# PimLb/POMDP_PBVI_Exploration

Measured on AMD Instinct MI355X. Metric: alpha-vector backups/sec, higher is better.
Workload: dtype f32

## Files before the change

include/pbvi_hip.h:

```cpp
#ifndef PBVI_HIP_H
#define PBVI_HIP_H

#include <stddef.h>
#include <stdint.h>

#ifdef __cplusplus
extern "C" {
#endif

typedef struct pbvi_engine pbvi_engine_t;

enum pbvi_status {
    PBVI_OK = 0,
    PBVI_EINVAL = -1,
    PBVI_ENOMEM = -2,
    PBVI_ERUNTIME = -3,
    PBVI_EUNSUPPORTED = -4
};

enum pbvi_dtype { PBVI_F32 = 0, PBVI_F64 = 1 };

enum pbvi_mode {
    PBVI_SPARSE = 0,
    PBVI_DENSE = 1
// ... 158 lines not shown
int pbvi_set_score_split(pbvi_engine_t* e, int mode);

int pbvi_set_gamma_tiling(pbvi_engine_t* e, int mode, int64_t chunk_rows);
int pbvi_gamma_tiling_plan(int32_t S, int32_t A, int32_t O, int64_t V, int64_t B, int dtype, int64_t budget_bytes,
                           int64_t* chunk_rows, int64_t* n_chunks, int64_t* bytes_needed);

int pbvi_set_tie_window(pbvi_engine_t* e, double rel);

int pbvi_debug_poison(int enable);
int64_t pbvi_debug_alloc_limit(int64_t mb);
int pbvi_engine_after_oom(pbvi_engine_t* e);
int64_t pbvi_debug_live_bytes(void);

int pbvi_debug_gemm_dense(int enable);
int pbvi_debug_split_schedule(int schedule);
int64_t pbvi_debug_slabs(pbvi_engine_t* e, void* out, int64_t cap_bytes);
int pbvi_debug_slabs_fill(pbvi_engine_t* e, int byte);

int64_t pbvi_device_bytes(const pbvi_engine_t* e);

#ifdef __cplusplus
}
#endif
#endif
```

pomdp_pbvi_exploration_amd/csrc/engine.hip:

```cpp
#include <algorithm>
#include <atomic>
#include <cmath>
#include <cstddef>
#include <cstdio>
#include <cstdlib>
#include <cstring>
#include <condition_variable>
#include <mutex>
#include <new>
#include <string>
#include <thread>
#include <unistd.h>
#include <vector>

#include "backup_kernels.h"
#include "split_bf16.h"

namespace pbvi {

static thread_local std::string g_err;
static int g_poison = -1;
static bool poison_enabled() {
    if (g_poison < 0) g_poison = getenv("PBVI_POISON") != nullptr ? 1 : 0;
    return g_poison == 1;
}
void set_error(const std::string& msg) { g_err = msg; }

#define HIPCHK(expr)                                                                         \
    do {                                                                                     \
        hipError_t _e = (expr);                                                              \
        if (_e != hipSuccess) {                                                              \
// ... 753 lines not shown
    virtual int store_select(int which, const int32_t* ids, int64_t n) = 0;
    virtual int store_reset(int which) = 0;
    virtual int after_oom() = 0;
    virtual int belief_update(const int32_t* act, const int32_t* obs, void* out) = 0;
    virtual int beliefs_advance(const int32_t* act, const int32_t* obs, const uint8_t* keep, int64_t* out_B) = 0;
    virtual int beliefs_fetch(void* out) = 0;
    virtual int set_rto_f64(const double* rto) = 0;
    virtual int64_t belief_walk(const double* b0, int64_t n, const int32_t* act, const int32_t* obs, const uint8_t* restart,
                                double* out) = 0;
    virtual int64_t beliefs_count() const = 0;
    virtual int walk_keys(int64_t n, uint64_t* out_keys) = 0;
    virtual int backup_value_max(double* out_value) = 0;
    virtual int q_values(double gamma, double* out_q, int32_t* out_action, int32_t* out_best) = 0;
    virtual int64_t debug_slabs(void* out, int64_t cap_bytes) = 0;
    virtual int debug_slabs_fill(int byte) = 0;
    virtual int rollout(int source, const int32_t* alpha_actions, double gamma, const int32_t* start_states,
                        const uint8_t* end_mask, uint64_t first_sim_id, uint64_t seed, int64_t T, int32_t* out_states,
                        int32_t* out_actions, int32_t* out_observations, int32_t* out_steps) = 0;
    virtual int infotaxis(double* out_g, int32_t* out_action, double* out_p_obs, double* out_entropy) = 0;
    virtual int env_set_frames(const uint8_t* frames, int64_t F, int64_t C, const int32_t* channel_of_action) = 0;
    virtual int env_set_table(const double* obs_prob) = 0;
    virtual int env_clear() = 0;
    virtual int rollout_env(int source, const int32_t* alpha_actions, double gamma, const int32_t* start_states,
                            const uint8_t* end_mask, int end_observation, const int64_t* shifts, uint64_t first_sim_id,
                            uint64_t seed, int64_t T, int32_t* out_states, int32_t* out_actions, int32_t* out_observations,
                            int32_t* out_steps, uint8_t* out_lost) = 0;
};

template <typename T>
class EngineT : public EngineBase {
// ... 105 lines not shown
    DevBuf e_bv_{mem_}, e_bs_{mem_}, e_err_{mem_}, e_rdot_{mem_}, e_act_{mem_}, e_ares_{mem_}, e_bres_{mem_}, e_rep_{mem_}, e_uniq_{mem_}, e_inv_{mem_}, e_slotd_{mem_}, e_cnt_{mem_, DevBuf::MODEL}, e_out_{mem_}, e_slot_{mem_};
    hipEvent_t ev_early_[2] = {nullptr, nullptr};
    hipEvent_t ev_ids_ = nullptr;
    hipEvent_t ev_nzA_ = nullptr;
    DevBuf nzBw_{mem_, DevBuf::MODEL};
    DevBuf nzB_{mem_, DevBuf::MODEL}, nzA_{mem_}, klist_{mem_}, kcount_{mem_}, nchunks_{mem_}, need_{mem_}, skws_{mem_};
    DevBuf dense_{mem_, DevBuf::MODEL}, nzD_{mem_, DevBuf::MODEL}, nzAlpha_{mem_}, prod_{mem_}, klistD_{mem_}, kcountD_{mem_}, nchunksD_{mem_};
    int64_t rows_pad_s_ = 0, dense_pairs_ = 0;
    std::vector<int> h_kcountD_;
    PinnedBuf kc_pin_{pinned_, "hipHostFree(kcount)"};
    hipStream_t stream2_ = nullptr;
    hipStream_t stream3_ = nullptr;
    hipEvent_t ev_fork_ = nullptr, ev_join_ = nullptr, ev_lists_ = nullptr, ev_xr_[2] = {nullptr, nullptr};
    GemmPlan plan_ = {};
    int64_t slab_bytes_ = 0;
    hipEvent_t ev_[9] = {};
    hipEvent_t ev_pg_[2] = {};
    bool have_result_ = false, res_sorted_ = false;
    int64_t res_B_ = 0;
    int screen_mode_ = 1;
    int split_mode_ = 1;
    bool split_supported_ = false;
    int fuse_project_ = 1;
    double irr_frac_ = 0.0;
    DevBuf irr_{mem_, DevBuf::MODEL};
    DevBuf mat_{mem_}, vlist_{mem_};
    DevBuf ctile_{mem_};
    std::vector<int32_t> h_ctile_;
    int n_mat_ = 0;
    bool gam_pad_compact_ = false;
// ... 772 lines not shown
            HIPCHK(hipStreamSynchronize(stream_));
        }
        return PBVI_OK;
    }

    int64_t debug_slabs(void* out, int64_t cap_bytes) override {
        if (slab_bytes_ <= 0 || slabs_.p == nullptr || (int64_t)slabs_.cap < slab_bytes_)
            FAIL(PBVI_EINVAL, "debug_slabs: no score GEMM has run");
        if (!out) return slab_bytes_;
        if (cap_bytes < slab_bytes_) FAIL(PBVI_EINVAL, "debug_slabs: the output array is smaller than the slab buffer");
        HIPCHK(hipSetDevice(device_));
        HIPCHK(hipMemcpyAsync(out, slabs_.p, (size_t)slab_bytes_, hipMemcpyDeviceToHost, stream_));
        HIPCHK(hipStreamSynchronize(stream_));
        return slab_bytes_;
    }
    int debug_slabs_fill(int byte) override {
        if (slab_bytes_ <= 0 || slabs_.p == nullptr || (int64_t)slabs_.cap < slab_bytes_)
            FAIL(PBVI_EINVAL, "debug_slabs_fill: no score GEMM has run");
        HIPCHK(hipSetDevice(device_));
        HIPCHK(hipMemsetAsync(slabs_.p, byte & 0xff, (size_t)slab_bytes_, stream_));
        HIPCHK(hipStreamSynchronize(stream_));
        return PBVI_OK;
    }

    int beliefs_fetch(void* out) override {
        if (B_ <= 0) FAIL(PBVI_EINVAL, "beliefs_fetch: no belief block resident");
        if (!out) FAIL(PBVI_EINVAL, "beliefs_fetch: NULL argument");
        HIPCHK(hipSetDevice(device_));
        if (!sorted_) {
            HIPCHK(hipMemcpy2DAsync(out, (size_t)S_ * sizeof(T), bel_.p, (size_t)S_pad_ * sizeof(T), (size_t)S_ * sizeof(T),
// ... 994 lines not shown
    }
    if constexpr (kF32) {
        const int64_t n_pad = round_up(rows_y, GEMM_BN);
        if (m_pad > 0x7fffffff || n_pad > 0x7fffffff) FAIL(PBVI_EUNSUPPORTED, "score_gemm: operand rows exceed int32");
        plan_ = make_gemm_plan((int)m_pad, (int)n_pad, S_pad_);
        const size_t pairs = (size_t)plan_.tiles_m * plan_.tiles_n;
        if ((rc = slabs_.ensure((size_t)plan_.c_floats * sizeof(float)))) return rc;
        slab_bytes_ = (int64_t)plan_.c_floats * (int64_t)sizeof(float);
        if ((rc = klist_.ensure(pairs * plan_.k_tiles * sizeof(int)))) return rc;
        if ((rc = kcount_.ensure(pairs * sizeof(int)))) return rc;
        if ((rc = nchunks_.ensure(pairs * sizeof(int)))) return rc;
        if ((rc = skws_.ensure(streamk_workspace_ints(plan_) * sizeof(int)))) return rc;
        int sp = split != nullptr && *split && plan_.streamk && (fused == nullptr || fused->R == 1) ? 1 : 0;
        if (sp && (!own_block || !split_plane())) sp = 0;
        if (split != nullptr) *split = sp;
        HIPCHK(launch_gemm_nt_f32(sp ? belsp_.as<float>() : (const float*)X, S_pad_, (const float*)Y, S_pad_, slabs_.as<float>(), plan_,
                                  nzX, nzB, G, v_group, (int)rows_y, klist_.as<int>(), kcount_.as<int>(),
                                  nchunks_.as<int>(), stream_, 1, 0, 0, skws_.as<int>(), list_stream, ev_lists_, nullptr, nullptr,
                                  fused, sp));
        sv->slabs = slabs_.as<T>();
        sv->slab_stride = plan_.slab_stride;
        sv->ldc = plan_.ldc;
        sv->nchunks = nchunks_.as<int>();
        sv->tiles_m = plan_.tiles_m;
        sv->fixed = 0;
        sv->first_block = plan_.streamk ? skws_.as<int>() + (pairs + 1) + plan_.nblocks : nullptr;
    } else {
        const int kt32s = S_pad_ / GEMM_BK;
        const int split = f64_uses_mfma(m_rows, rows_y) ? gemm_f64_split((int)m_rows, (int)rows_y, kt32s) : 1;
        if ((rc = slabs_.ensure((size_t)split * m_rows * rows_y * sizeof(T)))) return rc;
// ... 5 lines not shown
        } else {
            const int kt32 = S_pad_ / GEMM_BK;
            if ((rc = klist_.ensure(gemm_f64_klist_ints((int)m_rows, (int)rows_y, kt32) * sizeof(int)))) return rc;
            if ((rc = kcount_.ensure(gemm_f64_kcount_ints((int)m_rows, (int)rows_y, kt32) * sizeof(int)))) return rc;
            HIPCHK(launch_gemm_nt_f64((const double*)X, S_pad_, (int)m_rows, (const double*)Y, S_pad_, (int)rows_y,
                                      slabs_.as<double>(), (int)rows_y, S_pad_, nzX, nzB, G, v_group, klist_.as<int>(),
                                      kcount_.as<int>(), stream_, split, m_rows * rows_y));
            f64_pairs_ = (int64_t)gemm_f64_pairs((int)m_rows, (int)rows_y);
        }
        sv->slabs = slabs_.as<T>();
        sv->slab_stride = 0;
        sv->ldc = (int)rows_y;
        sv->nchunks = nullptr;
        sv->tiles_m = 0;
        sv->fixed = 1;
    }
    return PBVI_OK;
}

template <typename T>
int EngineT<T>::project_dense(double gamma) {
    int rc;
    const int AO = A_ * O_;
    const int64_t Vt = V_, Vt_pad = round_up(Vt, GEMM_BM);
    int64_t ld_prod, batch_stride;
    if constexpr (kF32) {
        const int64_t n_pad = rows_pad_s_;
        GemmPlan pl = make_gemm_plan((int)Vt_pad, (int)n_pad, S_pad_, true);
        const size_t pairs = (size_t)pl.tiles_m * pl.tiles_n;
        ld_prod = n_pad;
// ... 1283 lines not shown
void* pbvi_host_alloc(size_t bytes) {
    void* p = nullptr;
    if (bytes == 0) return nullptr;
    if (hipHostMalloc(&p, bytes, hipHostMallocDefault) != hipSuccess) {
        (void)hipGetLastError();
        pbvi::set_error("pbvi_host_alloc: hipHostMalloc of " + std::to_string(bytes) + " bytes failed");
        return nullptr;
    }
    return p;
}
void pbvi_host_free(void* p) {
    if (p && hipHostFree(p) != hipSuccess) (void)hipGetLastError();
}
int pbvi_debug_gemm_dense(int enable) { return pbvi::set_gemm_force_dense(enable); }
int pbvi_debug_split_schedule(int schedule) { return pbvi::set_gemm_split_schedule(schedule); }
int64_t pbvi_debug_slabs(pbvi_engine_t* e, void* out, int64_t cap_bytes) {
    NEED(e);
    return e->impl->debug_slabs(out, cap_bytes);
}
int pbvi_debug_slabs_fill(pbvi_engine_t* e, int byte) {
    NEED(e);
    return e->impl->debug_slabs_fill(byte);
}
int pbvi_backup(pbvi_engine_t* e, const void* beliefs, int64_t B, double gamma, int flags, void* out_alpha,
                int32_t* out_action, int32_t* out_best_alpha, uint8_t* out_keep, pbvi_stats_t* stats) {
    NEED(e);
    int rc = e->impl->beliefs_set(beliefs, B);
    if (rc) return rc;
    rc = e->impl->backup_run(gamma, flags, stats);
    if (rc) return rc;
// ... 183 lines not shown
```

pomdp_pbvi_exploration_amd/csrc/gemm.hip:

```cpp
#include "pbvi_common.h"
#include "split_bf16.h"

#include <cstdlib>
#include <map>
#include <mutex>

namespace pbvi {

typedef float f32x4 __attribute__((ext_vector_type(4)));
typedef float f32x16 __attribute__((ext_vector_type(16)));

constexpr int TILE_FLOATS = 256 * GEMM_BK;
constexpr int KL_IRR_BIT = 30;
constexpr int KL_MASK = (1 << KL_IRR_BIT) - 1;
constexpr int GEMM_LDS_BYTES = 4 * TILE_FLOATS * 4;

__device__ __forceinline__ void glds16(const float* g, float* l) {
    __builtin_amdgcn_global_load_lds((const __attribute__((address_space(1))) void*)g,
                                     (__attribute__((address_space(3))) void*)l, 16, 0, 0);
}

struct TileThread {
    int lane, wid, i, h, wr, wc;
    int srow[4], scol[4];
// ... 872 lines not shown
            if (more) store_b(buf ^ 1, 1);
            split_group(t, lds, buf, 1, 2, f, acc);
        }
        asm volatile("s_waitcnt vmcnt(0)" : "+v"(idx[0]), "+v"(idx[1])::"memory");
        __syncthreads();
        buf ^= 1;
        k_next = k_after;
        k_after = k_after2;
    }
}

template <int SCHED>
__device__ __forceinline__ void gemm_split_streamk_body(
    const float* __restrict__ A, int lda, const float* __restrict__ B, int ldb, FusedB fb, float* __restrict__ C, int ldc,
    int64_t slab_stride, int tiles_m, int pairs, int k_tiles, const int* __restrict__ klist, const int* __restrict__ kcount,
    const int* __restrict__ prefix, const int* __restrict__ start_pair, const int* __restrict__ first_block,
    const int* __restrict__ plan, int ovh) {
    extern __shared__ __attribute__((aligned(16))) float lds[];
    const int nb = gridDim.x;
    int L;
    {
        const int bid = blockIdx.x, xcd = bid & 7, qq = nb >> 3, r = nb & 7;
        const int base = (xcd < r) ? xcd * (qq + 1) : r * (qq + 1) + (xcd - r) * qq;
        L = base + (bid >> 3);
    }
    const int q = plan[0], T = plan[1];
    int64_t pos = (int64_t)L * q;
    if (pos >= T) return;
    const int64_t end = (pos + q < T) ? pos + q : T;
    int p = start_pair[L];
    if (p < 0) return;
    TileThread t;
    t.init();
    while (pos < end && p < pairs) {
        const int cnt = kcount[p];
        if (cnt == 0) {
            ++p;
            continue;
        }
        const int u_lo = (int)(pos - prefix[p]);
        const int64_t room = end - pos;
        const int u_hi = (u_lo + room < cnt + ovh) ? (int)(u_lo + room) : cnt + ovh;
        const int lo = u_lo > ovh ? u_lo - ovh : 0;
        const int hi = u_hi > ovh ? u_hi - ovh : 0;
        if (hi > lo) {
            const int tm = p % tiles_m, tn = p / tiles_m;
            f32x16 acc[4][2];
            tile_zero(acc);
            const float* Ablk = A + (int64_t)tm * 256 * lda;
            if (fb.mat == nullptr || fb.mat[tn]) {
                const int bt = (fb.mat != nullptr && fb.ctile != nullptr) ? fb.ctile[tn] : tn;
                tile_run_split<SCHED>(t, lds, Ablk, lda, B + (int64_t)bt * 256 * ldb, ldb, false, nullptr, nullptr, nullptr, 0,
                                      0.f, klist + (int64_t)p * k_tiles, lo, hi, acc);
            } else {
                const int r0 = tn * 256;
                const int g = r0 / fb.V, v0 = r0 - g * fb.V;
                tile_run_split<SCHED>(t, lds, Ablk, lda, nullptr, 0, true, fb.rs + (int64_t)(g / fb.O) * fb.S_pad,
                                      fb.rto + (int64_t)g * fb.S_pad, fb.alpha + (int64_t)(v0 + (threadIdx.x >> 2)) * fb.lda,
                                      (int64_t)128 * fb.lda, fb.gamma, klist + (int64_t)p * k_tiles, lo, hi, acc);
            }
            const bool cont = L != first_block[p];
            tile_store(t, cont ? C + slab_stride + (int64_t)L * (256 * 256) : C, cont ? 256 : ldc, cont ? 0 : tm, cont ? 0 : tn, acc);
        }
        pos += u_hi - u_lo;
        ++p;
    }
}

#define PBVI_SPLIT_KERNEL_ARGS                                                                                              \
    const float *__restrict__ A, int lda, const float *__restrict__ B, int ldb, FusedB fb, float *__restrict__ C, int ldc,      \
        int64_t slab_stride, int tiles_m, int pairs, int k_tiles, const int *__restrict__ klist,                               \
        const int *__restrict__ kcount, const int *__restrict__ prefix, const int *__restrict__ start_pair,                    \
        const int *__restrict__ first_block, const int *__restrict__ plan, int ovh
__global__ __launch_bounds__(512) void k_gemm_split_streamk(PBVI_SPLIT_KERNEL_ARGS) {
    gemm_split_streamk_body<SPLIT_SCHED_PARENT>(A, lda, B, ldb, fb, C, ldc, slab_stride, tiles_m, pairs, k_tiles, klist, kcount,
                                                prefix, start_pair, first_block, plan, ovh);
}
__global__ __launch_bounds__(512) void k_gemm_split_streamk_pipelined(PBVI_SPLIT_KERNEL_ARGS) {
    gemm_split_streamk_body<SPLIT_SCHED_PIPELINED>(A, lda, B, ldb, fb, C, ldc, slab_stride, tiles_m, pairs, k_tiles, klist, kcount,
                                                   prefix, start_pair, first_block, plan, ovh);
}
#undef PBVI_SPLIT_KERNEL_ARGS

__global__ void k_split_probe(float* out) {
    const int lane = threadIdx.x, r = lane & 31, h = lane >> 5;
    float a[8] = {0.f, 0.f, 0.f, 0.f, 0.f, 0.f, 0.f, 0.f}, b[8] = {0.f, 0.f, 0.f, 0.f, 0.f, 0.f, 0.f, 0.f};
    const float x = 0x1.02p-120f + 0x1p-132f;
    if (h == 0) {
        a[0] = x;
        a[1] = 0x1p-100f;
        if (r == 0) b[0] = 1.f;
        if (r == 1) b[1] = 0x1p-30f;
    }
    i32x4 ah, al, bh, bl;
    uint32_t hh, ll;
#pragma unroll
    for (int p = 0; p < 4; ++p) {
// ... 115 lines not shown
int gemm_force_dense() {
    if (g_force_dense < 0) g_force_dense = getenv("PBVI_GEMM_DENSE") ? (atoi(getenv("PBVI_GEMM_DENSE")) != 0) : 0;
    return g_force_dense;
}
int set_gemm_force_dense(int enable) {
    const int prev = gemm_force_dense();
    g_force_dense = enable ? 1 : 0;
    return prev;
}

static int g_split_schedule = SPLIT_SCHED_PARENT;
int set_gemm_split_schedule(int schedule) {
    const int prev = g_split_schedule;
    if (schedule == SPLIT_SCHED_PARENT || schedule == SPLIT_SCHED_PIPELINED) g_split_schedule = schedule;
    return prev;
}

int choose_chunk_len(int tiles_mn, int k_tiles) {
    if (const char* env = getenv("PBVI_GEMM_CHUNK")) {
        const int v = atoi(env);
        if (v > 0) return v < k_tiles ? v : k_tiles;
    }
    const int64_t total = (int64_t)tiles_mn * k_tiles;
    int64_t len = total / (256 * 8);
    if (len < 8) len = 8;
    if (len > 96) len = 96;
    if (len > k_tiles) len = k_tiles;
    return (int)len;
}

// ... 53 lines not shown
    const int force_dense = gemm_force_dense();
    hipStream_t ls = (list_stream != nullptr && list_event != nullptr) ? list_stream : stream;
    if (fused != nullptr && !pl.streamk) return hipErrorInvalidValue;
    if (split && (!pl.streamk || (fused != nullptr && fused->R != 1))) return hipErrorInvalidValue;
    hipLaunchKernelGGL(k_build_klists, dim3(pairs, batch), dim3(256), 0, ls, nzA, nzB, G, v_group, n_rows,
                       pl.tiles_m, pl.k_tiles, pl.chunk_len, force_dense, klist, kcount, nchunks,
                       fused != nullptr ? fused->irr : nullptr, fused != nullptr ? fused->O : 1);
    e = hipGetLastError();
    if (e != hipSuccess) return e;
    if (pl.streamk) {
        if (batch != 1 || streamk_ws == nullptr) return hipErrorInvalidValue;
        int* prefix = streamk_ws;
        int* start_pair = prefix + pairs + 1;
        int* first_block = start_pair + pl.nblocks;
        int* plan = first_block + pairs;
        static const int ovh = getenv("PBVI_STREAMK_OVH") ? atoi(getenv("PBVI_STREAMK_OVH")) : 1;
        hipLaunchKernelGGL(k_streamk_plan, dim3(1), dim3(256), 0, ls, kcount, pairs, pl.nblocks, pl.k_tiles,
                           pl.max_chunks - 1, ovh, prefix, start_pair, first_block, nchunks, plan);
        e = hipGetLastError();
        if (e != hipSuccess) return e;
        if (ls != stream) {
            if ((e = hipEventRecord(list_event, ls)) != hipSuccess) return e;
            if ((e = hipStreamWaitEvent(stream, list_event, 0)) != hipSuccess) return e;
        }
        if (split) {
            FusedB fb{};
            if (fused != nullptr) fb = *fused;
            hipLaunchKernelGGL(g_split_schedule == SPLIT_SCHED_PIPELINED ? k_gemm_split_streamk_pipelined : k_gemm_split_streamk,
                               dim3(pl.nblocks), dim3(512), GEMM_LDS_BYTES, stream, A, lda, B, ldb, fb, C, pl.ldc, pl.slab_stride,
                               pl.tiles_m, pairs, pl.k_tiles, klist, kcount, prefix, start_pair, first_block, plan, ovh);
        } else if (fused != nullptr && fused->R > 1) {
            switch (fused->R) {
#define PBVI_FUSED_R_CASE(RR)                                                                                                   \
    case RR:                                                                                                                    \
        hipLaunchKernelGGL(k_gemm_nt_f32_streamk_fused_r<RR>, dim3(pl.nblocks), dim3(512), GEMM_LDS_BYTES_R, stream, A, lda, B, \
                           ldb, *fused, C, pl.ldc, pl.slab_stride, pl.tiles_m, pairs, pl.k_tiles, klist, kcount, prefix,        \
                           start_pair, first_block, plan, ovh);                                                                 \
        break;
                PBVI_FUSED_R_CASE(2) PBVI_FUSED_R_CASE(3) PBVI_FUSED_R_CASE(4) PBVI_FUSED_R_CASE(5) PBVI_FUSED_R_CASE(6) PBVI_FUSED_R_CASE(7)
#undef PBVI_FUSED_R_CASE
                default:
                    return hipErrorInvalidValue;
            }
        } else if (fused != nullptr)
            hipLaunchKernelGGL(k_gemm_nt_f32_streamk_fused, dim3(pl.nblocks), dim3(512), GEMM_LDS_BYTES, stream, A, lda, B, ldb,
// ... 38 lines not shown
        const int max_split = 8;
        pl.chunk_len = pl.k_tiles;
        pl.max_chunks = max_split + 1;
        pl.c_floats = pl.slab_stride + (int64_t)pl.nblocks * (256 * 256);
        return pl;
    } else {
        pl.chunk_len = choose_chunk_len(pl.tiles_m * pl.tiles_n, pl.k_tiles);
        pl.max_chunks = (pl.k_tiles + pl.chunk_len - 1) / pl.chunk_len;
    }
    pl.c_floats = (int64_t)pl.max_chunks * pl.slab_stride;
    return pl;
}

size_t streamk_workspace_ints(const GemmPlan& pl) {
    const size_t pairs = (size_t)pl.tiles_m * pl.tiles_n;
    return (pairs + 1) + (size_t)pl.nblocks + pairs + 2;
}

template <typename T>
__global__ void k_gemm_nt_simple(const T* __restrict__ A, int lda, const T* __restrict__ B, int ldb,
                                 T* __restrict__ C, int ldc, int M, int N, int K) {
    __shared__ T As[16][17];
    __shared__ T Bs[16][17];
    const int tx = threadIdx.x, ty = threadIdx.y;
    const int m = blockIdx.y * 16 + ty, n = blockIdx.x * 16 + tx;
    T acc = 0;
    for (int k0 = 0; k0 < K; k0 += 16) {
        const int ka = k0 + tx;
        const int ma = blockIdx.y * 16 + ty, nb = blockIdx.x * 16 + ty;
        As[ty][tx] = (ma < M && ka < K) ? A[(int64_t)ma * lda + ka] : T(0);
        Bs[ty][tx] = (nb < N && ka < K) ? B[(int64_t)nb * ldb + ka] : T(0);
// ... 22 lines not shown
```

pomdp_pbvi_exploration_amd/csrc/pbvi_common.h:

```cpp
#pragma once
#include <hip/hip_runtime.h>
#include <stdint.h>
#include <string>

#include "../../include/pbvi_hip.h"

namespace pbvi {

void set_error(const std::string& msg);

constexpr int GEMM_BM = 256;
constexpr int GEMM_BN = 256;
constexpr int GEMM_BK = 32;

inline int64_t round_up(int64_t x, int64_t m) { return (x + m - 1) / m * m; }

struct GemmPlan {
    int tiles_m, tiles_n, k_tiles, chunk_len, max_chunks, ldc;
    int64_t slab_stride;
    bool streamk;
    int nblocks;
    int64_t c_floats;
};
int set_gemm_force_dense(int enable);
int set_gemm_split_schedule(int schedule);
int gemm_force_dense();
size_t streamk_workspace_ints(const GemmPlan& pl);
struct FusedB {
    const float* alpha;
    int lda;
    const int32_t* rs;
    const float* rto;
    int S_pad, O, V;
    int R;
    float gamma;
    const int32_t* ctile;
    const uint8_t* mat;
    const int32_t* irr;
};
GemmPlan make_gemm_plan(int M_pad, int N_pad, int K_pad, bool single_chunk = false);
// ... 32 lines not shown
```

pomdp_pbvi_exploration_amd/engine.py:

```python
from __future__ import annotations

import ctypes as C
import os
from dataclasses import dataclass

import numpy as np

PKG_DIR = os.path.dirname(os.path.abspath(__file__))
LIB_PATH = os.path.join(PKG_DIR, 'libpbvi_hip.so')

PBVI_F32, PBVI_F64 = 0, 1
PBVI_SPARSE, PBVI_DENSE = 0, 1
PBVI_BELIEF_DOMINANCE = 1

EXPORTS = [
    'pbvi_version', 'pbvi_device_count', 'pbvi_last_error', 'pbvi_engine_create', 'pbvi_engine_destroy',
    'pbvi_alpha_set', 'pbvi_alpha_append', 'pbvi_alpha_count', 'pbvi_beliefs_set', 'pbvi_backup_run',
    'pbvi_backup_fetch', 'pbvi_backup_unique_count', 'pbvi_backup_fetch_unique', 'pbvi_backup_device_results',
    'pbvi_backup', 'pbvi_prune_dominated', 'pbvi_value_max',
    'pbvi_set_tie_window', 'pbvi_device_bytes',
    'pbvi_alpha_store_append', 'pbvi_alpha_select', 'pbvi_alpha_store_reset',
    'pbvi_belief_store_append', 'pbvi_beliefs_select', 'pbvi_belief_store_reset', 'pbvi_debug_poison',
    'pbvi_belief_update', 'pbvi_beliefs_advance', 'pbvi_beliefs_fetch', 'pbvi_beliefs_count',
    'pbvi_mdp_value_iteration', 'pbvi_set_formulation', 'pbvi_belief_walk', 'pbvi_engine_set_rto_f64', 'pbvi_backup_fetch_unique_keys', 'pbvi_assemble_rows',
    'pbvi_backup_fetch_exchange', 'pbvi_backup_store_unique',
    'pbvi_value_max_store', 'pbvi_belief_store_count', 'pbvi_alpha_store_count', 'pbvi_set_value_max_exact', 'pbvi_alpha_layout',
    'pbvi_belief_walk_keys', 'pbvi_backup_fetch_value_max',
    'pbvi_backup_fetch_compact', 'pbvi_host_alloc', 'pbvi_host_free', 'pbvi_debug_gemm_dense',
    'pbvi_backup_fetch_exchange_padded', 'pbvi_assemble_rows_store', 'pbvi_exchange_merge', 'pbvi_backup_run_fetch', 'pbvi_debug_alloc_limit', 'pbvi_debug_live_bytes', 'pbvi_engine_after_oom', 'pbvi_set_f64_screen', 'pbvi_set_fused_projection', 'pbvi_backup_fetch_row_hashes', 'pbvi_set_score_split',
    'pbvi_set_gamma_tiling', 'pbvi_gamma_tiling_plan', 'pbvi_q_values', 'pbvi_prune_dominated_masked',
    'pbvi_rollout', 'pbvi_infotaxis', 'pbvi_rollout_infotaxis', 'pbvi_debug_split_schedule', 'pbvi_debug_slabs',
    'pbvi_debug_slabs_fill', 'pbvi_env_set_frames', 'pbvi_env_set_table', 'pbvi_env_clear', 'pbvi_rollout_env',
]


class EngineUnavailable(RuntimeError):
    """The HIP library is missing or no GPU is visible."""


class PbviStats(C.Structure):
    _fields_ = [('ms_total', C.c_double), ('ms_project', C.c_double), ('ms_score', C.c_double),
                ('ms_argmax', C.c_double), ('ms_refine', C.c_double), ('ms_action', C.c_double),
                ('ms_assemble', C.c_double), ('ms_dominance', C.c_double), ('n_pairs', C.c_int64),
                ('n_dead', C.c_int64), ('n_refined', C.c_int64), ('n_refined_actions', C.c_int64),
                ('n_unique', C.c_int64),
                ('score_flops', C.c_int64), ('score_flops_executed', C.c_int64), ('score_tiles_dense', C.c_int64),
                ('score_tiles_run', C.c_int64), ('project_flops', C.c_int64), ('project_flops_executed', C.c_int64),
# ... 29 lines not shown
                                         i32p, vp, vp, C.c_int, C.c_int]),
        'pbvi_engine_destroy': (None, [vp]),
        'pbvi_alpha_set': (C.c_int, [vp, vp, C.c_int64]),
        'pbvi_alpha_append': (C.c_int, [vp, vp, C.c_int64]),
        'pbvi_alpha_count': (C.c_int64, [vp]),
        'pbvi_beliefs_set': (C.c_int, [vp, vp, C.c_int64]),
        'pbvi_backup_run': (C.c_int, [vp, C.c_double, C.c_int, sp]),
        'pbvi_backup_fetch': (C.c_int, [vp, vp, i32p, i32p, u8p]),
        'pbvi_backup_unique_count': (C.c_int64, [vp]),
        'pbvi_backup_fetch_unique': (C.c_int, [vp, vp, i32p]),
        'pbvi_backup_fetch_compact': (C.c_int, [vp, vp, i32p, i32p, i32p, u8p]),
        'pbvi_host_alloc': (vp, [C.c_size_t]),
        'pbvi_host_free': (None, [vp]),
        'pbvi_debug_gemm_dense': (C.c_int, [C.c_int]),
        'pbvi_debug_split_schedule': (C.c_int, [C.c_int]),
        'pbvi_debug_slabs': (C.c_int64, [vp, vp, C.c_int64]),
        'pbvi_debug_slabs_fill': (C.c_int, [vp, C.c_int]),
        'pbvi_backup_store_unique': (C.c_int64, [vp, i32p, C.c_int64]),
        'pbvi_backup_device_results': (C.c_int, [vp, C.POINTER(vp), C.POINTER(vp), C.POINTER(vp)]),
        'pbvi_backup': (C.c_int, [vp, vp, C.c_int64, C.c_double, C.c_int, vp, i32p, i32p, u8p, sp]),
        'pbvi_prune_dominated': (C.c_int, [vp, u8p]),
        'pbvi_prune_dominated_masked': (C.c_int, [vp, u8p, u8p]),
        'pbvi_value_max': (C.c_int, [vp, f64p, i32p]),
        'pbvi_value_max_store': (C.c_int, [vp, C.c_int64, f64p, i32p]),
        'pbvi_q_values': (C.c_int, [vp, C.c_double, f64p, i32p, i32p]),
        'pbvi_belief_store_count': (C.c_int64, [vp]),
        'pbvi_backup_fetch_value_max': (C.c_int, [vp, f64p]),
        'pbvi_belief_walk_keys': (C.c_int, [vp, C.c_int64, C.POINTER(C.c_uint64)]),
        'pbvi_set_value_max_exact': (C.c_int, [vp, C.c_int]),
        'pbvi_alpha_layout': (C.c_int, [vp, C.POINTER(C.c_int64), C.POINTER(C.c_int64)]),
# ... 77 lines not shown
    return int(rows.value), int(n.value), int(need.value)


def debug_gemm_dense(enable: bool) -> bool:
    return bool(load_library().pbvi_debug_gemm_dense(1 if enable else 0))


SPLIT_SCHEDULES = {'parent': 0, 'pipelined': 1}


def debug_split_schedule(schedule: str) -> str:
    prev = int(load_library().pbvi_debug_split_schedule(SPLIT_SCHEDULES[schedule]))
    return {v: k for k, v in SPLIT_SCHEDULES.items()}[prev]


def device_count() -> int:
    return int(load_library().pbvi_device_count())


class _PinnedArray(np.ndarray):

    def __array_finalize__(self, obj):
        self._owner = getattr(obj, '_owner', None)


class PinnedBuffer:

    def __init__(self, nbytes: int):
        self._lib = load_library()
        self.nbytes = int(nbytes)
# ... 901 lines not shown
        self._ck(self._lib.pbvi_set_f64_screen(self._h, {'off': 0, 'auto': 1, 'always': 2}[mode]))

    def set_score_split(self, mode: str = 'auto') -> None:
        self._ck(self._lib.pbvi_set_score_split(self._h, {'off': 0, 'auto': 1, 'always': 2}[mode]))

    def debug_slabs(self) -> np.ndarray:
        n = int(self._lib.pbvi_debug_slabs(self._h, None, 0))
        if n < 0:
            self._ck(n)
        out = np.empty(n, dtype=np.uint8)
        got = int(self._lib.pbvi_debug_slabs(self._h, _ptr(out), n))
        if got < 0:
            self._ck(got)
        return out

    def debug_slabs_fill(self, byte: int) -> None:
        self._ck(self._lib.pbvi_debug_slabs_fill(self._h, int(byte)))

    def set_gamma_tiling(self, mode: str = 'off', chunk_rows: int = 0) -> None:
        self._ck(self._lib.pbvi_set_gamma_tiling(self._h, {'off': 0, 'auto': 1, 'always': 2}[mode], int(chunk_rows)))
        self._gamma_tiling = (mode, int(chunk_rows))

    @property
    def gamma_tiling(self) -> tuple:
        if self._gamma_tiling is None:
            mode, _, rows = os.environ.get('PBVI_GAMMA_TILING', '').partition(':')
            mode = {'auto': 'auto', '1': 'auto', 'always': 'always', '2': 'always'}.get(mode, 'off')
            self._gamma_tiling = (mode, max(0, int(rows)) if rows.lstrip('-').isdigit() else 0)
        return self._gamma_tiling

# ... 7 lines not shown
```

Before: 657,300.

## Add gang-aware stream-K planner mapping planes to XCD-grouped blocks

Replaces the split stream-K planning kernel with a multi-phase planner that can group identical output planes into gangs and map them onto blocks that share an XCD, using explicit walk order, share boundaries and a logical-of-block table. The GEMM kernel now reads per-block share ranges and a walk permutation instead of computing uniform shares inline. The gang mode is off by default, so the default path keeps the old partitioning through new tables, with extra indirection and a larger planning kernel. Debug hooks are added to inspect the plan.

```diff
diff --git a/include/pbvi_hip.h b/include/pbvi_hip.h
--- a/include/pbvi_hip.h
+++ b/include/pbvi_hip.h
@@ -196,6 +196,9 @@
 
 int pbvi_debug_gemm_dense(int enable);
 int pbvi_debug_split_schedule(int schedule);
+int pbvi_debug_streamk_gangs(int enable);
+int pbvi_debug_streamk_plan(pbvi_engine_t* e, int32_t* dims, int32_t* share_begin, int32_t* walk, int32_t* logical_of_bid,
+                            int32_t* first_block, int32_t* nchunks, int32_t* kcount, int32_t* plan);
 int64_t pbvi_debug_slabs(pbvi_engine_t* e, void* out, int64_t cap_bytes);
 int pbvi_debug_slabs_fill(pbvi_engine_t* e, int byte);
 
diff --git a/pomdp_pbvi_exploration_amd/csrc/engine.hip b/pomdp_pbvi_exploration_amd/csrc/engine.hip
--- a/pomdp_pbvi_exploration_amd/csrc/engine.hip
+++ b/pomdp_pbvi_exploration_amd/csrc/engine.hip
@@ -15,6 +15,7 @@
 
 #include "backup_kernels.h"
 #include "split_bf16.h"
+#include "streamk_plan.h"
 
 namespace pbvi {
 
@@ -798,6 +799,8 @@
     virtual int q_values(double gamma, double* out_q, int32_t* out_action, int32_t* out_best) = 0;
     virtual int64_t debug_slabs(void* out, int64_t cap_bytes) = 0;
     virtual int debug_slabs_fill(int byte) = 0;
+    virtual int debug_streamk_plan(int32_t* dims, int32_t* share_begin, int32_t* walk, int32_t* logical_of_bid, int32_t* first_block,
+                                   int32_t* nchunks, int32_t* kcount, int32_t* plan) = 0;
     virtual int rollout(int source, const int32_t* alpha_actions, double gamma, const int32_t* start_states,
                         const uint8_t* end_mask, uint64_t first_sim_id, uint64_t seed, int64_t T, int32_t* out_states,
                         int32_t* out_actions, int32_t* out_observations, int32_t* out_steps) = 0;
@@ -933,6 +936,8 @@
     hipEvent_t ev_fork_ = nullptr, ev_join_ = nullptr, ev_lists_ = nullptr, ev_xr_[2] = {nullptr, nullptr};
     GemmPlan plan_ = {};
     int64_t slab_bytes_ = 0;
+    bool split_plan_ = false;
+    int split_G_ = 0, split_V_ = 0;
     hipEvent_t ev_[9] = {};
     hipEvent_t ev_pg_[2] = {};
     bool have_result_ = false, res_sorted_ = false;
@@ -1735,6 +1740,33 @@
         HIPCHK(hipStreamSynchronize(stream_));
         return slab_bytes_;
     }
+    int debug_streamk_plan(int32_t* dims, int32_t* share_begin, int32_t* walk, int32_t* logical_of_bid, int32_t* first_block,
+                           int32_t* nchunks, int32_t* kcount, int32_t* plan) override {
+        if constexpr (!kF32) {
+            FAIL(PBVI_EINVAL, "debug_streamk_plan: no split score GEMM has run");
+        } else {
+            if (!split_plan_ || !plan_.streamk || skws_.p == nullptr) FAIL(PBVI_EINVAL, "debug_streamk_plan: no split score GEMM has run");
+            if (!dims) FAIL(PBVI_EINVAL, "debug_streamk_plan: NULL argument");
+            const size_t pairs = (size_t)plan_.tiles_m * plan_.tiles_n, nb = (size_t)plan_.nblocks;
+            const int32_t d[10] = {(int32_t)pairs, plan_.nblocks, plan_.tiles_m, plan_.tiles_n, plan_.k_tiles, split_G_, split_V_,
+                                   plan_.max_chunks - 1, streamk_ovh(), SK_PLAN_WORDS};
+            for (int i = 0; i < 10; ++i) dims[i] = d[i];
+            const int* ws = skws_.as<int>();
+            const int* d_first = ws + (pairs + 1) + nb;
+            const int* d_plan = d_first + pairs;
+            const int* d_share = d_plan + SK_PLAN_WORDS;
+            const int* d_walk = d_share + nb + 1;
+            const int* d_lob = d_walk + pairs;
+            HIPCHK(hipSetDevice(device_));
+            const struct { int32_t* dst; const int* src; size_t n; } copies[7] = {
+                {share_begin, d_share, nb + 1}, {walk, d_walk, pairs}, {logical_of_bid, d_lob, nb}, {first_block, d_first, pairs},
+                {nchunks, nchunks_.as<int>(), pairs}, {kcount, kcount_.as<int>(), pairs}, {plan, d_plan, (size_t)SK_PLAN_WORDS}};
+            for (const auto& c : copies)
+                if (c.dst) HIPCHK(hipMemcpyAsync(c.dst, c.src, c.n * sizeof(int32_t), hipMemcpyDeviceToHost, stream_));
+            HIPCHK(hipStreamSynchronize(stream_));
+            return PBVI_OK;
+        }
+    }
     int debug_slabs_fill(int byte) override {
         if (slab_bytes_ <= 0 || slabs_.p == nullptr || (int64_t)slabs_.cap < slab_bytes_)
             FAIL(PBVI_EINVAL, "debug_slabs_fill: no score GEMM has run");
@@ -2759,6 +2791,9 @@
         int sp = split != nullptr && *split && plan_.streamk && (fused == nullptr || fused->R == 1) ? 1 : 0;
         if (sp && (!own_block || !split_plane())) sp = 0;
         if (split != nullptr) *split = sp;
+        split_plan_ = sp != 0;
+        split_G_ = G;
+        split_V_ = v_group;
         HIPCHK(launch_gemm_nt_f32(sp ? belsp_.as<float>() : (const float*)X, S_pad_, (const float*)Y, S_pad_, slabs_.as<float>(), plan_,
                                   nzX, nzB, G, v_group, (int)rows_y, klist_.as<int>(), kcount_.as<int>(),
                                   nchunks_.as<int>(), stream_, 1, 0, 0, skws_.as<int>(), list_stream, ev_lists_, nullptr, nullptr,
@@ -2794,6 +2829,7 @@
         sv->nchunks = nullptr;
         sv->tiles_m = 0;
         sv->fixed = 1;
+        split_plan_ = false;
     }
     return PBVI_OK;
 }
@@ -4107,6 +4143,12 @@
 }
 int pbvi_debug_gemm_dense(int enable) { return pbvi::set_gemm_force_dense(enable); }
 int pbvi_debug_split_schedule(int schedule) { return pbvi::set_gemm_split_schedule(schedule); }
+int pbvi_debug_streamk_gangs(int enable) { return pbvi::set_gemm_streamk_gangs(enable); }
+int pbvi_debug_streamk_plan(pbvi_engine_t* e, int32_t* dims, int32_t* share_begin, int32_t* walk, int32_t* logical_of_bid,
+                            int32_t* first_block, int32_t* nchunks, int32_t* kcount, int32_t* plan) {
+    NEED(e);
+    return e->impl->debug_streamk_plan(dims, share_begin, walk, logical_of_bid, first_block, nchunks, kcount, plan);
+}
 int64_t pbvi_debug_slabs(pbvi_engine_t* e, void* out, int64_t cap_bytes) {
     NEED(e);
     return e->impl->debug_slabs(out, cap_bytes);
diff --git a/pomdp_pbvi_exploration_amd/csrc/gemm.hip b/pomdp_pbvi_exploration_amd/csrc/gemm.hip
--- a/pomdp_pbvi_exploration_amd/csrc/gemm.hip
+++ b/pomdp_pbvi_exploration_amd/csrc/gemm.hip
@@ -1,5 +1,6 @@
 #include "pbvi_common.h"
 #include "split_bf16.h"
+#include "streamk_plan.h"
 
 #include <cstdlib>
 #include <map>
@@ -910,28 +911,22 @@
 __device__ __forceinline__ void gemm_split_streamk_body(
     const float* __restrict__ A, int lda, const float* __restrict__ B, int ldb, FusedB fb, float* __restrict__ C, int ldc,
     int64_t slab_stride, int tiles_m, int pairs, int k_tiles, const int* __restrict__ klist, const int* __restrict__ kcount,
-    const int* __restrict__ prefix, const int* __restrict__ start_pair, const int* __restrict__ first_block,
-    const int* __restrict__ plan, int ovh) {
+    const int* __restrict__ prefix, const int* __restrict__ start_pos, const int* __restrict__ first_block,
+    const int* __restrict__ share_begin, const int* __restrict__ walk, const int* __restrict__ logical_of_bid, int ovh) {
     extern __shared__ __attribute__((aligned(16))) float lds[];
-    const int nb = gridDim.x;
-    int L;
-    {
-        const int bid = blockIdx.x, xcd = bid & 7, qq = nb >> 3, r = nb & 7;
-        const int base = (xcd < r) ? xcd * (qq + 1) : r * (qq + 1) + (xcd - r) * qq;
-        L = base + (bid >> 3);
-    }
-    const int q = plan[0], T = plan[1];
-    int64_t pos = (int64_t)L * q;
-    if (pos >= T) return;
-    const int64_t end = (pos + q < T) ? pos + q : T;
-    int p = start_pair[L];
-    if (p < 0) return;
+    const int L = logical_of_bid[blockIdx.x];
+    int64_t pos = share_begin[L];
+    const int64_t end = share_begin[L + 1];
+    if (pos >= end) return;
+    int w = start_pos[L];
+    if (w < 0) return;
     TileThread t;
     t.init();
-    while (pos < end && p < pairs) {
+    while (pos < end && w < pairs) {
+        const int p = walk[w];
         const int cnt = kcount[p];
         if (cnt == 0) {
-            ++p;
+            ++w;
             continue;
         }
         const int u_lo = (int)(pos - prefix[p]);
@@ -959,24 +954,35 @@
             tile_store(t, cont ? C + slab_stride + (int64_t)L * (256 * 256) : C, cont ? 256 : ldc, cont ? 0 : tm, cont ? 0 : tn, acc);
         }
         pos += u_hi - u_lo;
-        ++p;
+        ++w;
     }
 }
 
 #define PBVI_SPLIT_KERNEL_ARGS                                                                                              \
     const float *__restrict__ A, int lda, const float *__restrict__ B, int ldb, FusedB fb, float *__restrict__ C, int ldc,      \
         int64_t slab_stride, int tiles_m, int pairs, int k_tiles, const int *__restrict__ klist,                               \
-        const int *__restrict__ kcount, const int *__restrict__ prefix, const int *__restrict__ start_pair,                    \
-        const int *__restrict__ first_block, const int *__restrict__ plan, int ovh
+        const int *__restrict__ kcount, const int *__restrict__ prefix, const int *__restrict__ start_pos,                     \
+        const int *__restrict__ first_block, const int *__restrict__ share_begin, const int *__restrict__ walk,                \
+        const int *__restrict__ logical_of_bid, int ovh
 __global__ __launch_bounds__(512) void k_gemm_split_streamk(PBVI_SPLIT_KERNEL_ARGS) {
     gemm_split_streamk_body<SPLIT_SCHED_PARENT>(A, lda, B, ldb, fb, C, ldc, slab_stride, tiles_m, pairs, k_tiles, klist, kcount,
-                                                prefix, start_pair, first_block, plan, ovh);
+                                                prefix, start_pos, first_block, share_begin, walk, logical_of_bid, ovh);
 }
 __global__ __launch_bounds__(512) void k_gemm_split_streamk_pipelined(PBVI_SPLIT_KERNEL_ARGS) {
     gemm_split_streamk_body<SPLIT_SCHED_PIPELINED>(A, lda, B, ldb, fb, C, ldc, slab_stride, tiles_m, pairs, k_tiles, klist, kcount,
-                                                   prefix, start_pair, first_block, plan, ovh);
+                                                   prefix, start_pos, first_block, share_begin, walk, logical_of_bid, ovh);
 }
 #undef PBVI_SPLIT_KERNEL_ARGS
+
+__global__ __launch_bounds__(SK_PLAN_THREADS) void k_streamk_gang_plan(SkPlanArgs a) {
+    __shared__ SkScratch s;
+    const int tid = threadIdx.x;
+#define PBVI_SK_RUN(phase) \
+    phase(tid, a, s);      \
+    __syncthreads();
+    PBVI_SK_PHASES(PBVI_SK_RUN)
+#undef PBVI_SK_RUN
+}
 
 __global__ void k_split_probe(float* out) {
     const int lane = threadIdx.x, r = lane & 31, h = lane >> 5;
@@ -1122,6 +1128,22 @@
     const int prev = g_split_schedule;
     if (schedule == SPLIT_SCHED_PARENT || schedule == SPLIT_SCHED_PIPELINED) g_split_schedule = schedule;
     return prev;
+}
+
+constexpr int STREAMK_GANGS_DEFAULT = 0;
+static int g_streamk_gangs = -1;
+static int streamk_gangs() {
+    if (g_streamk_gangs < 0) g_streamk_gangs = getenv("PBVI_STREAMK_GANGS") ? (atoi(getenv("PBVI_STREAMK_GANGS")) != 0) : STREAMK_GANGS_DEFAULT;
+    return g_streamk_gangs;
+}
+int set_gemm_streamk_gangs(int enable) {
+    const int prev = streamk_gangs();
+    g_streamk_gangs = enable ? 1 : 0;
+    return prev;
+}
+int streamk_ovh() {
+    static const int ovh = getenv("PBVI_STREAMK_OVH") ? atoi(getenv("PBVI_STREAMK_OVH")) : 1;
+    return ovh;
 }
 
 int choose_chunk_len(int tiles_mn, int k_tiles) {
@@ -1205,9 +1227,39 @@
         int* start_pair = prefix + pairs + 1;
         int* first_block = start_pair + pl.nblocks;
         int* plan = first_block + pairs;
-        static const int ovh = getenv("PBVI_STREAMK_OVH") ? atoi(getenv("PBVI_STREAMK_OVH")) : 1;
-        hipLaunchKernelGGL(k_streamk_plan, dim3(1), dim3(256), 0, ls, kcount, pairs, pl.nblocks, pl.k_tiles,
-                           pl.max_chunks - 1, ovh, prefix, start_pair, first_block, nchunks, plan);
+        int* share_begin = plan + SK_PLAN_WORDS;
+        int* walk = share_begin + pl.nblocks + 1;
+        int* logical_of_bid = walk + pairs;
+        int* wcost = logical_of_bid + pl.nblocks;
+        const int ovh = streamk_ovh();
+        if (split) {
+            SkPlanArgs a{};
+            a.kcount = kcount;
+            a.pairs = pairs;
+            a.tiles_m = pl.tiles_m;
+            a.tiles_n = pl.tiles_n;
+            a.nblocks = pl.nblocks;
+            a.k_tiles = pl.k_tiles;
+            a.max_split = pl.max_chunks - 1;
+            a.ovh = ovh;
+            a.G = G;
+            a.V = v_group;
+            a.n_rows = n_rows;
+            a.gangs = streamk_gangs();
+            a.prefix = prefix;
+            a.start_pos = start_pair;
+            a.first_block = first_block;
+            a.nchunks = nchunks;
+            a.plan = plan;
+            a.share_begin = share_begin;
+            a.walk = walk;
+            a.logical_of_bid = logical_of_bid;
+            a.wcost = wcost;
+            hipLaunchKernelGGL(k_streamk_gang_plan, dim3(1), dim3(SK_PLAN_THREADS), 0, ls, a);
+        } else {
+            hipLaunchKernelGGL(k_streamk_plan, dim3(1), dim3(256), 0, ls, kcount, pairs, pl.nblocks, pl.k_tiles,
+                               pl.max_chunks - 1, ovh, prefix, start_pair, first_block, nchunks, plan);
+        }
         e = hipGetLastError();
         if (e != hipSuccess) return e;
         if (ls != stream) {
@@ -1219,7 +1271,8 @@
             if (fused != nullptr) fb = *fused;
             hipLaunchKernelGGL(g_split_schedule == SPLIT_SCHED_PIPELINED ? k_gemm_split_streamk_pipelined : k_gemm_split_streamk,
                                dim3(pl.nblocks), dim3(512), GEMM_LDS_BYTES, stream, A, lda, B, ldb, fb, C, pl.ldc, pl.slab_stride,
-                               pl.tiles_m, pairs, pl.k_tiles, klist, kcount, prefix, start_pair, first_block, plan, ovh);
+                               pl.tiles_m, pairs, pl.k_tiles, klist, kcount, prefix, start_pair, first_block, share_begin, walk,
+                               logical_of_bid, ovh);
         } else if (fused != nullptr && fused->R > 1) {
             switch (fused->R) {
 #define PBVI_FUSED_R_CASE(RR)                                                                                                   \
@@ -1288,7 +1341,7 @@
 
 size_t streamk_workspace_ints(const GemmPlan& pl) {
     const size_t pairs = (size_t)pl.tiles_m * pl.tiles_n;
-    return (pairs + 1) + (size_t)pl.nblocks + pairs + 2;
+    return (pairs + 1) + (size_t)pl.nblocks + pairs + SK_PLAN_WORDS + ((size_t)pl.nblocks + 1) + pairs + (size_t)pl.nblocks + pairs;
 }
 
 template <typename T>
diff --git a/pomdp_pbvi_exploration_amd/csrc/pbvi_common.h b/pomdp_pbvi_exploration_amd/csrc/pbvi_common.h
--- a/pomdp_pbvi_exploration_amd/csrc/pbvi_common.h
+++ b/pomdp_pbvi_exploration_amd/csrc/pbvi_common.h
@@ -24,6 +24,8 @@
 };
 int set_gemm_force_dense(int enable);
 int set_gemm_split_schedule(int schedule);
+int set_gemm_streamk_gangs(int enable);
+int streamk_ovh();
 int gemm_force_dense();
 size_t streamk_workspace_ints(const GemmPlan& pl);
 struct FusedB {
diff --git a/pomdp_pbvi_exploration_amd/csrc/streamk_plan.h b/pomdp_pbvi_exploration_amd/csrc/streamk_plan.h
--- /dev/null
+++ b/pomdp_pbvi_exploration_amd/csrc/streamk_plan.h
@@ -0,0 +1,312 @@
+#pragma once
+#include <stdint.h>
+
+#if defined(__HIPCC__)
+#define PBVI_HD __host__ __device__ inline
+#else
+#define PBVI_HD inline
+#endif
+
+namespace pbvi {
+
+constexpr int SK_PLAN_THREADS = 256;
+constexpr int SK_MAX_PLANES = 16;
+enum { SKP_QMAX = 0, SKP_T = 1, SKP_P = 2, SKP_NB_PLANE = 3, SKP_Q_PLANE = 4, SKP_Q_REM = 5, SKP_T_PLANE = 6, SKP_PLANE_PAIRS = 7, SK_PLAN_WORDS = 8 };
+
+struct SkShares {
+    int P;
+    int nb_plane;
+    int nb_rem;
+    int q_plane, q_rem;
+    int T_plane, T_rem;
+};
+
+struct SkPlanArgs {
+    const int* kcount;
+    int pairs, tiles_m, tiles_n, nblocks, k_tiles, max_split, ovh;
+    int G, V;
+    int64_t n_rows;
+    int gangs;
+    int *prefix;
+    int *start_pos;
+    int *first_block;
+    int *nchunks;
+    int *plan;
+    int *share_begin;
+    int *walk;
+    int *logical_of_bid;
+    int *wcost;
+};
+
+struct SkScratch {
+    int part[SK_PLAN_THREADS], part_plane[SK_PLAN_THREADS], ok[SK_PLAN_THREADS];
+    int red[SK_PLAN_THREADS / 16], red_plane[SK_PLAN_THREADS / 16], red_ok[SK_PLAN_THREADS / 16];
+    int P0;
+    SkShares sh;
+};
+
+PBVI_HD int sk_cost(int cnt, int ovh) { return cnt > 0 ? cnt + ovh : 0; }
+PBVI_HD int sk_first_inside(int g, int V) { return (int)(((unsigned)g * (unsigned)V + 255u) >> 8); }
+PBVI_HD bool sk_tile_inside(int tn, int G, int V) {
+    const unsigned r0 = (unsigned)tn * 256u, r1 = r0 + 255u;
+    return r1 < (unsigned)G * (unsigned)V && r0 / (unsigned)V == r1 / (unsigned)V;
+}
+
+PBVI_HD int sk_gang_planes(int G, int V, int64_t n_rows, int tiles_n, int nblocks) {
+    if (G <= 0 || V <= 0 || nblocks <= 0 || (nblocks & 7) != 0) return 0;
+    if (n_rows < (int64_t)G * V || (int64_t)tiles_n * 256 < (int64_t)G * V || (int64_t)tiles_n * 256 > 0x7fffffff) return 0;
+    if (V < 2 * 256) return 0;
+    int C = SK_MAX_PLANES;
+    for (int g = 0; g < G && C >= 2; ++g) {
+        const int c = (int)(((unsigned)(g + 1) * (unsigned)V) >> 8) - sk_first_inside(g, V);
+        if (c < C) C = c < 0 ? 0 : c;
+    }
+    if (C > (nblocks >> 3)) C = nblocks >> 3;
+    int P = 1;
+    while (2 * P <= C) P *= 2;
+    return P >= 2 ? P : 0;
+}
+
+PBVI_HD int sk_plane_pair(int j, int i, int tiles_m, int V) {
+    const int g = i / tiles_m, tm = i - g * tiles_m;
+    return (sk_first_inside(g, V) + j) * tiles_m + tm;
+}
+
+PBVI_HD int sk_walk_pos(int p, int P, int G, int V, int tiles_m) {
+    if (P == 0) return p;
+    const int tn = p / tiles_m, tm = p - tn * tiles_m;
+    const int plane_pairs = G * tiles_m;
+    const unsigned r0 = (unsigned)tn * 256u;
+    int before;
+    if (r0 >= (unsigned)G * (unsigned)V) {
+        before = P * G;
+    } else {
+        const int g = (int)(r0 / (unsigned)V);
+        const int d = tn - sk_first_inside(g, V);
+        if (d < P && sk_tile_inside(tn, G, V)) return d * plane_pairs + g * tiles_m + tm;
+        before = P * g + (d < P ? d : P);
+    }
+    return P * plane_pairs + (p - before * tiles_m);
+}
+
+PBVI_HD int sk_q(int64_t cost, int blocks, int qmin) {
+    int64_t q = blocks > 0 ? (cost + blocks - 1) / blocks : 0;
+    if (q < qmin) q = qmin;
+    if (q < 1) q = 1;
+    return (int)q;
+}
+
+PBVI_HD SkShares sk_shares(int P0, int64_t T_plane, int64_t T, int nblocks, int qmin) {
+    SkShares sh;
+    sh.P = 0;
+    sh.nb_plane = 0;
+    sh.nb_rem = nblocks;
+    sh.T_plane = 0;
+    sh.T_rem = (int)T;
+    sh.q_rem = sk_q(T, nblocks, qmin);
+    sh.q_plane = sh.q_rem;
+    if (P0 < 2 || T_plane <= 0 || T <= 0) return sh;
+    const int64_t T_rem = T - (int64_t)P0 * T_plane;
+    if (T_rem < 0) return sh;
+    const int cap_xcd = 8 * ((nblocks >> 3) / P0);
+    const int cap_rem = (nblocks - (T_rem > 0 ? 1 : 0)) / P0;
+    const int cap = cap_xcd < cap_rem ? cap_xcd : cap_rem;
+    if (cap < 1) return sh;
+    const int64_t num = (int64_t)nblocks * T_plane;
+    int cand[2] = {(int)(num / T), (int)((num + T - 1) / T)};
+    int best = 0, best_q = 0;
+    for (int c = 0; c < 2; ++c) {
+        int nb = cand[c];
+        if (nb < 1) nb = 1;
+        if (nb > cap) nb = cap;
+        const int qp = sk_q(T_plane, nb, qmin), qr = sk_q(T_rem, nblocks - P0 * nb, qmin);
+        const int qm = qp > qr ? qp : qr;
+        if (best == 0 || qm < best_q) {
+            best = nb;
+            best_q = qm;
+        }
+    }
+    sh.P = P0;
+    sh.nb_plane = best;
+    sh.nb_rem = nblocks - P0 * best;
+    sh.T_plane = (int)T_plane;
+    sh.T_rem = (int)T_rem;
+    sh.q_plane = sk_q(T_plane, best, qmin);
+    sh.q_rem = sk_q(T_rem, sh.nb_rem, qmin);
+    return sh;
+}
+
+PBVI_HD int sk_share_begin(int L, const SkShares& sh) {
+    const int nbp = sh.P * sh.nb_plane;
+    if (L < nbp) {
+        const int j = (int)((unsigned)L / (unsigned)sh.nb_plane), s = L - j * sh.nb_plane;
+        const int64_t off = (int64_t)s * sh.q_plane;
+        return j * sh.T_plane + (off < sh.T_plane ? (int)off : sh.T_plane);
+    }
+    const int64_t off = (int64_t)(L - nbp) * sh.q_rem;
+    return sh.P * sh.T_plane + (off < sh.T_rem ? (int)off : sh.T_rem);
+}
+
+PBVI_HD int sk_block_of(int x, const SkShares& sh) {
+    const int pt = sh.P * sh.T_plane;
+    if (x < pt) {
+        const unsigned j = (unsigned)x / (unsigned)sh.T_plane, r = (unsigned)x - j * (unsigned)sh.T_plane;
+        return (int)(j * (unsigned)sh.nb_plane + r / (unsigned)sh.q_plane);
+    }
+    return sh.P * sh.nb_plane + (int)((unsigned)(x - pt) / (unsigned)sh.q_rem);
+}
+
+PBVI_HD int sk_gang_slots(int xcd, const SkShares& sh) { return xcd < sh.nb_plane ? sh.P * ((sh.nb_plane - xcd + 7) >> 3) : 0; }
+PBVI_HD int sk_logical_of_bid(int bid, int nblocks, const SkShares& sh) {
+    const int xcd = bid & 7, slot = bid >> 3;
+    if (sh.P == 0) {
+        const int qq = nblocks >> 3, r = nblocks & 7;
+        const int base = (xcd < r) ? xcd * (qq + 1) : r * (qq + 1) + (xcd - r) * qq;
+        return base + slot;
+    }
+    const int per_xcd = nblocks >> 3, used = sk_gang_slots(xcd, sh);
+    if (slot < used) {
+        const int k = (int)((unsigned)slot / (unsigned)sh.P), j = slot - k * sh.P;
+        return j * sh.nb_plane + k * 8 + xcd;
+    }
+    int r = slot - used;
+    for (int x = 0; x < xcd; ++x) r += per_xcd - sk_gang_slots(x, sh);
+    return sh.P * sh.nb_plane + r;
+}
+
+PBVI_HD void sk_phase_sums(int tid, const SkPlanArgs& a, SkScratch& s) {
+    const int P0 = a.gangs ? sk_gang_planes(a.G, a.V, a.n_rows, a.tiles_n, a.nblocks) : 0;
+    if (tid == 0) s.P0 = P0;
+    int sum = 0, sum_plane = 0, ok = 1;
+    for (int p = tid; p < a.pairs; p += SK_PLAN_THREADS) sum += sk_cost(a.kcount[p], a.ovh);
+    if (P0 > 0) {
+        const int plane_pairs = a.G * a.tiles_m;
+        for (int i = tid; i < plane_pairs; i += SK_PLAN_THREADS) {
+            const int c0 = a.kcount[sk_plane_pair(0, i, a.tiles_m, a.V)];
+            sum_plane += sk_cost(c0, a.ovh);
+            for (int j = 1; j < P0; ++j)
+                if (a.kcount[sk_plane_pair(j, i, a.tiles_m, a.V)] != c0) ok = 0;
+        }
+    }
+    s.part[tid] = sum;
+    s.part_plane[tid] = sum_plane;
+    s.ok[tid] = ok;
+}
+
+PBVI_HD void sk_phase_reduce(int tid, const SkPlanArgs&, SkScratch& s) {
+    if (tid >= SK_PLAN_THREADS / 16) return;
+    int sum = 0, sum_plane = 0, ok = 1;
+    for (int i = 16 * tid; i < 16 * tid + 16; ++i) {
+        sum += s.part[i];
+        sum_plane += s.part_plane[i];
+        ok &= s.ok[i];
+    }
+    s.red[tid] = sum;
+    s.red_plane[tid] = sum_plane;
+    s.red_ok[tid] = ok;
+}
+
+PBVI_HD void sk_phase_shares(int tid, const SkPlanArgs& a, SkScratch& s) {
+    if (tid != 0) return;
+    int64_t T = 0, T_plane = 0;
+    int ok = 1;
+    for (int i = 0; i < SK_PLAN_THREADS / 16; ++i) {
+        T += s.red[i];
+        T_plane += s.red_plane[i];
+        ok &= s.red_ok[i];
+    }
+    const int qmin = (a.k_tiles + a.ovh + a.max_split - 1) / a.max_split;
+    s.sh = sk_shares(ok ? s.P0 : 0, T_plane, T, a.nblocks, qmin);
+    a.plan[SKP_QMAX] = s.sh.q_plane > s.sh.q_rem ? s.sh.q_plane : s.sh.q_rem;
+    a.plan[SKP_T] = (int)T;
+    a.plan[SKP_P] = s.sh.P;
+    a.plan[SKP_NB_PLANE] = s.sh.nb_plane;
+    a.plan[SKP_Q_PLANE] = s.sh.q_plane;
+    a.plan[SKP_Q_REM] = s.sh.q_rem;
+    a.plan[SKP_T_PLANE] = s.sh.T_plane;
+    a.plan[SKP_PLANE_PAIRS] = s.sh.P > 0 ? a.G * a.tiles_m : 0;
+    a.prefix[a.pairs] = (int)T;
+}
+
+PBVI_HD void sk_phase_tables(int tid, const SkPlanArgs& a, SkScratch& s) {
+    for (int p = tid; p < a.pairs; p += SK_PLAN_THREADS) {
+        const int w = sk_walk_pos(p, s.sh.P, a.G, a.V, a.tiles_m);
+        a.walk[w] = p;
+        a.wcost[w] = sk_cost(a.kcount[p], a.ovh);
+    }
+    for (int i = tid; i < a.nblocks; i += SK_PLAN_THREADS) {
+        a.start_pos[i] = -1;
+        a.logical_of_bid[i] = sk_logical_of_bid(i, a.nblocks, s.sh);
+    }
+    for (int i = tid; i <= a.nblocks; i += SK_PLAN_THREADS) a.share_begin[i] = sk_share_begin(i, s.sh);
+}
+
+PBVI_HD void sk_chunk(int tid, int pairs, int& w0, int& w1) {
+    const int per = (pairs + SK_PLAN_THREADS - 1) / SK_PLAN_THREADS;
+    w0 = (int64_t)tid * per < pairs ? tid * per : pairs;
+    w1 = w0 + per < pairs ? w0 + per : pairs;
+}
+
+PBVI_HD void sk_phase_chunk_sums(int tid, const SkPlanArgs& a, SkScratch& s) {
+    int w0, w1, sum = 0;
+    sk_chunk(tid, a.pairs, w0, w1);
+    for (int w = w0; w < w1; ++w) sum += a.wcost[w];
+    s.part[tid] = sum;
+}
+
+PBVI_HD void sk_phase_scan_runs(int tid, const SkPlanArgs&, SkScratch& s) {
+    if (tid >= SK_PLAN_THREADS / 16) return;
+    int run = 0;
+    for (int i = 16 * tid; i < 16 * tid + 16; ++i) {
+        const int v = s.part[i];
+        s.part[i] = run;
+        run += v;
+    }
+    s.red[tid] = run;
+}
+
+PBVI_HD void sk_phase_scan_totals(int tid, const SkPlanArgs&, SkScratch& s) {
+    if (tid != 0) return;
+    int run = 0;
+    for (int i = 0; i < SK_PLAN_THREADS / 16; ++i) {
+        const int v = s.red[i];
+        s.red[i] = run;
+        run += v;
+    }
+}
+
+PBVI_HD void sk_phase_pairs(int tid, const SkPlanArgs& a, SkScratch& s) {
+    int w0, w1;
+    sk_chunk(tid, a.pairs, w0, w1);
+    int run = s.part[tid] + s.red[tid >> 4];
+    for (int w = w0; w < w1; ++w) {
+        const int p = a.walk[w];
+        const int cost = a.wcost[w];
+        a.prefix[p] = run;
+        if (cost > 0) {
+            const int fb = sk_block_of(run, s.sh), lb = sk_block_of(run + cost - 1, s.sh);
+            const int fw = sk_block_of(run + a.ovh, s.sh);
+            a.first_block[p] = fw;
+            a.nchunks[p] = lb - fw + 1;
+            for (int i = fb; i <= lb; ++i)
+                if (sk_share_begin(i, s.sh) >= run) a.start_pos[i] = w;
+            run += cost;
+        } else {
+            a.first_block[p] = 0;
+            a.nchunks[p] = 0;
+        }
+    }
+}
+
+#define PBVI_SK_PHASES(X)                                                                                           \
+    X(sk_phase_sums) X(sk_phase_reduce) X(sk_phase_shares) X(sk_phase_tables) X(sk_phase_chunk_sums) X(sk_phase_scan_runs) \
+    X(sk_phase_scan_totals) X(sk_phase_pairs)
+
+inline void sk_plan_host(const SkPlanArgs& a, SkScratch& s) {
+#define PBVI_SK_RUN(phase) \
+    for (int tid = 0; tid < SK_PLAN_THREADS; ++tid) phase(tid, a, s);
+    PBVI_SK_PHASES(PBVI_SK_RUN)
+#undef PBVI_SK_RUN
+}
+
+}
diff --git a/pomdp_pbvi_exploration_amd/engine.py b/pomdp_pbvi_exploration_amd/engine.py
--- a/pomdp_pbvi_exploration_amd/engine.py
+++ b/pomdp_pbvi_exploration_amd/engine.py
@@ -31,6 +31,7 @@
     'pbvi_set_gamma_tiling', 'pbvi_gamma_tiling_plan', 'pbvi_q_values', 'pbvi_prune_dominated_masked',
     'pbvi_rollout', 'pbvi_infotaxis', 'pbvi_rollout_infotaxis', 'pbvi_debug_split_schedule', 'pbvi_debug_slabs',
     'pbvi_debug_slabs_fill', 'pbvi_env_set_frames', 'pbvi_env_set_table', 'pbvi_env_clear', 'pbvi_rollout_env',
+    'pbvi_debug_streamk_gangs', 'pbvi_debug_streamk_plan',
 ]
 
 
@@ -90,6 +91,8 @@
         'pbvi_host_free': (None, [vp]),
         'pbvi_debug_gemm_dense': (C.c_int, [C.c_int]),
         'pbvi_debug_split_schedule': (C.c_int, [C.c_int]),
+        'pbvi_debug_streamk_gangs': (C.c_int, [C.c_int]),
+        'pbvi_debug_streamk_plan': (C.c_int, [vp, i32p, i32p, i32p, i32p, i32p, i32p, i32p, i32p]),
         'pbvi_debug_slabs': (C.c_int64, [vp, vp, C.c_int64]),
         'pbvi_debug_slabs_fill': (C.c_int, [vp, C.c_int]),
         'pbvi_backup_store_unique': (C.c_int64, [vp, i32p, C.c_int64]),
@@ -197,6 +200,10 @@
     return {v: k for k, v in SPLIT_SCHEDULES.items()}[prev]
 
 
+def debug_streamk_gangs(enable: bool) -> bool:
+    return bool(load_library().pbvi_debug_streamk_gangs(1 if enable else 0))
+
+
 def device_count() -> int:
     return int(load_library().pbvi_device_count())
 
@@ -1128,6 +1135,21 @@
             self._ck(got)
         return out
 
+    def debug_streamk_plan(self) -> dict:
+        i32p = C.POINTER(C.c_int32)
+        none = C.cast(None, i32p)
+        dims = np.zeros(10, dtype=np.int32)
+        self._ck(self._lib.pbvi_debug_streamk_plan(self._h, dims.ctypes.data_as(i32p), none, none, none, none, none, none, none))
+        out = dict(zip(('pairs', 'nblocks', 'tiles_m', 'tiles_n', 'k_tiles', 'G', 'V', 'max_split', 'ovh', 'plan_words'),
+                       (int(x) for x in dims)))
+        sizes = {'share_begin': out['nblocks'] + 1, 'walk': out['pairs'], 'logical_of_bid': out['nblocks'],
+                 'first_block': out['pairs'], 'nchunks': out['pairs'], 'kcount': out['pairs'], 'plan': out['plan_words']}
+        arrays = {k: np.zeros(n, dtype=np.int32) for k, n in sizes.items()}
+        self._ck(self._lib.pbvi_debug_streamk_plan(self._h, dims.ctypes.data_as(i32p),
+                                                   *[a.ctypes.data_as(i32p) for a in arrays.values()]))
+        out.update(arrays)
+        return out
+
     def debug_slabs_fill(self, byte: int) -> None:
         self._ck(self._lib.pbvi_debug_slabs_fill(self._h, int(byte)))
 
```

Result: no change. 656,000, median of 3 (-0.2%).
